# CarluerJB/3D_SIFT_CUDA

Measured on AMD Instinct MI355X. Metric: keypoints/s (.key records per second; Gauss-pyramid GB/s vs HBM roofline in `pyramid`/`roofline`), higher is better.
Workload: dtype f32

## Files before the change

### 3d_sift_cuda_amd/csrc/kernels_keypoint.hip

```cpp
#include <cstddef>
#include <type_traits>

#include "sift3d_internal.h"

#define PD SIFT3D_PATCH_DIM
#define PV SIFT3D_PATCH_VOX


__device__ __forceinline__ void interp_coord(float fX, float fMin, float fMax, int &ix, float &w)
{
    if (fX < fMin + 0.5f) {
        ix = (int)fMin;
        w = 1.0f;
    } else if (fX >= fMax - 0.5f) {
        ix = (int)(fMax - 2);
        w = 0.0f;
    } else {
        float mh = fX - 0.5f;
        ix = (int)floorf(mh);
        w = 1.0f - (mh - ((float)ix));
    }
}

__device__ __forceinline__ float trilinear(const float *__restrict__ img, int X, int XP, int Y, int Z, int Zl, int z_off,
                                           float x, float y, float z)
{
    float wx, wy, wz;
    int ix, iy, iz;
    interp_coord(x, 0, (float)X, ix, wx);
    interp_coord(y, 0, (float)Y, iy, wy);
    interp_coord(z, 0, (float)Z, iz, wz);
    iz -= z_off;
    iz = iz < 0 ? 0 : (iz > Zl - 2 ? Zl - 2 : iz);
    const long long XY = (long long)XP * Y;
    const float *p = img + (long long)iz * XY + (long long)iy * XP + ix;
    typedef float f2u __attribute__((ext_vector_type(2), aligned(4)));
    const f2u q00 = *reinterpret_cast<const f2u *>(p), q10 = *reinterpret_cast<const f2u *>(p + XP);
    const f2u q01 = *reinterpret_cast<const f2u *>(p + XY), q11 = *reinterpret_cast<const f2u *>(p + XY + XP);
    const float f000 = q00.x, f100 = q00.y, f010 = q10.x, f110 = q10.y;
    const float f001 = q01.x, f101 = q01.y, f011 = q11.x, f111 = q11.y;
    float fn00 = wx * f000 + (1.0f - wx) * f100;
    float fn01 = wx * f001 + (1.0f - wx) * f101;
    float fn10 = wx * f010 + (1.0f - wx) * f110;
    float fn11 = wx * f011 + (1.0f - wx) * f111;
    float fnn0 = wy * fn00 + (1.0f - wy) * fn10;
    float fnn1 = wy * fn01 + (1.0f - wy) * fn11;
    return wz * fnn0 + (1.0f - wz) * fnn1;
}

__device__ __forceinline__ double finddet(double a1, double a2, double a3, double b1, double b2, double b3, double c1,
                                          double c2, double c3)
{
    return ((a1 * b2 * c3) - (a1 * b3 * c2) - (a2 * b1 * c3) + (a3 * b1 * c2) + (a2 * b3 * c1) - (a3 * b2 * c1));
}
__device__ __forceinline__ double interp_quadratic(double x0, double x1, double x2, double fx0, double fx1, double fx2)
{
    if (!(fx1 < fx0 && fx1 < fx2) && !(fx1 > fx0 && fx1 > fx2)) return x1;
    double a1 = x0 * x0, b1 = x0, c1 = 1;
    double a2 = x1 * x1, b2 = x1, c2 = 1;
    double a3 = x2 * x2, b3 = x2, c3 = 1;
    double d1 = fx0, d2 = fx1, d3 = fx2;
    double det = finddet(a1, a2, a3, b1, b2, b3, c1, c2, c3);
    double detx = finddet(d1, d2, d3, b1, b2, b3, c1, c2, c3);
    double dety = finddet(a1, a2, a3, d1, d2, d3, c1, c2, c3);
    if (d1 == 0 && d2 == 0 && d3 == 0) return x1;
    if (det != 0) {
        if (detx != 0) return dety / (-2.0 * detx);
    }
    return x1;
}

__device__ __forceinline__ void invert3(const float *in, float *out)
{
    float a11 = in[0], a21 = in[3], a31 = in[6];
    float a12 = in[1], a22 = in[4], a32 = in[7];
    float a13 = in[2], a23 = in[5], a33 = in[8];
    float det = a11 * (a33 * a22 - a32 * a23) - a21 * (a33 * a12 - a32 * a13) + a31 * (a23 * a12 - a22 * a13);
    double div = 1 / (double)det;
    out[0] = (float)((a33 * a22 - a32 * a23) * div);
    out[3] = (float)(-(a33 * a21 - a31 * a23) * div);
    out[6] = (float)((a32 * a21 - a31 * a22) * div);
    out[1] = (float)(-(a33 * a12 - a32 * a13) * div);
    out[4] = (float)((a33 * a11 - a31 * a13) * div);
    out[7] = (float)(-(a32 * a11 - a31 * a12) * div);
    out[2] = (float)((a23 * a12 - a22 * a13) * div);
    out[5] = (float)(-(a23 * a11 - a21 * a13) * div);
    out[8] = (float)((a22 * a11 - a21 * a12) * div);
}

__device__ __forceinline__ void v3_norm(float *p)
{
    float ss = p[0] * p[0] + p[1] * p[1] + p[2] * p[2];
    if (ss > 0) {
        float div = (float)(1.0 / (double)sqrtf(ss));
        p[0] *= div;
        p[1] *= div;
        p[2] *= div;
    } else {
        p[0] = 1;
        p[1] = 0;
        p[2] = 0;
    }
}
__device__ __forceinline__ float v3_mag(const float *p)
{
    float ss = p[0] * p[0] + p[1] * p[1] + p[2] * p[2];
    if (ss > 0) return sqrtf(ss);
    return 0;
}
__device__ __forceinline__ float v3_dot(const float *a, const float *b) { return a[0] * b[0] + a[1] * b[1] + a[2] * b[2]; }

__device__ __forceinline__ double svd_with_sign(double magnitude, double sign_source) { return sign_source >= 0.0 ? fabs(magnitude) : -fabs(magnitude); }
__device__ __forceinline__ double svd_hypot(double p, double q) { return sqrt(p * p + q * q); }

__device__ __forceinline__ void svd3(float a[3][3], float w[3], float v[3][3])
{
    double off[3];
    double g = 0.0, scale = 0.0, norm = 0.0, s, f, h;
    int below = 0;

    for (int i = 0; i < 3; i++) {
        below = i + 1;
        off[i] = scale * g;
        g = s = scale = 0.0;
        for (int k = i; k < 3; k++) scale += fabsf(a[k][i]);
        if (scale) {
            for (int k = i; k < 3; k++) {
                a[k][i] = (float)(a[k][i] / scale);
                s += a[k][i] * a[k][i];
            }
            f = a[i][i];
            g = -svd_with_sign(sqrt(s), f);
            h = f * g - s;
            a[i][i] = (float)(f - g);
            for (int j = below; j < 3; j++) {
                s = 0.0;
                for (int k = i; k < 3; k++) s += a[k][i] * a[k][j];
                f = s / h;
                for (int k = i; k < 3; k++) a[k][j] = (float)(a[k][j] + f * a[k][i]);
            }
            for (int k = i; k < 3; k++) a[k][i] = (float)(a[k][i] * scale);
        }
        w[i] = (float)(scale * g);
        g = s = scale = 0.0;
        if (i != 2) {
            for (int k = below; k < 3; k++) scale += fabsf(a[i][k]);
            if (scale) {
                for (int k = below; k < 3; k++) {
                    a[i][k] = (float)(a[i][k] / scale);
                    s += a[i][k] * a[i][k];
                }
                f = a[i][below];
                g = -svd_with_sign(sqrt(s), f);
                h = f * g - s;
                a[i][below] = (float)(f - g);
                for (int k = below; k < 3; k++) off[k] = a[i][k] / h;
                for (int j = below; j < 3; j++) {
                    s = 0.0;
                    for (int k = below; k < 3; k++) s += a[j][k] * a[i][k];
                    for (int k = below; k < 3; k++) a[j][k] = (float)(a[j][k] + s * off[k]);
                }
                for (int k = below; k < 3; k++) a[i][k] = (float)(a[i][k] * scale);
            }
        }
        const double row_norm = fabsf(w[i]) + fabs(off[i]);
        norm = norm > row_norm ? norm : row_norm;
    }

    for (int i = 2; i >= 0; i--) {
        if (i < 2) {
            if (g) {
                for (int j = below; j < 3; j++) v[j][i] = (float)((a[i][j] / a[i][below]) / g);
                for (int j = below; j < 3; j++) {
                    s = 0.0;
                    for (int k = below; k < 3; k++) s += a[i][k] * v[k][j];
                    for (int k = below; k < 3; k++) v[k][j] = (float)(v[k][j] + s * v[k][i]);
                }
            }
            for (int j = below; j < 3; j++) v[i][j] = v[j][i] = 0.0;
        }
        v[i][i] = 1.0;
        g = off[i];
        below = i;
    }

    for (int i = 2; i >= 0; i--) {
        below = i + 1;
        g = w[i];
        for (int j = below; j < 3; j++) a[i][j] = 0.0;
        if (g) {
            g = 1.0 / g;
            for (int j = below; j < 3; j++) {
                s = 0.0;
                for (int k = below; k < 3; k++) s += a[k][i] * a[k][j];
                f = (s / a[i][i]) * g;
                for (int k = i; k < 3; k++) a[k][j] = (float)(a[k][j] + f * a[k][i]);
            }
            for (int j = i; j < 3; j++) a[j][i] = (float)(a[j][i] * g);
        } else {
            for (int j = i; j < 3; j++) a[j][i] = 0.0;
        }
        a[i][i] = a[i][i] + 1;
    }

    for (int k = 2; k >= 0; k--) {
        for (int sweep = 1; sweep <= 30; sweep++) {
            bool cancel = true;
            int lo = k, above = 0;
            for (; lo >= 0; lo--) {
                above = lo - 1;
                if ((double)(fabs(off[lo]) + norm) == norm) {
                    cancel = false;
                    break;
                }
                if ((double)(fabsf(w[above]) + norm) == norm) break;
            }
            double c, x, y, z;
            if (cancel) {
                c = 0.0;
                s = 1.0;
                for (int i = lo; i <= k; i++) {
                    f = s * off[i];
                    off[i] = c * off[i];
                    if ((double)(fabs(f) + norm) == norm) break;
                    g = w[i];
                    h = svd_hypot(f, g);
                    w[i] = (float)h;
                    h = 1.0 / h;
                    c = g * h;
                    s = -f * h;
                    for (int j = 0; j < 3; j++) {
                        y = a[j][above];
                        z = a[j][i];
                        a[j][above] = (float)(y * c + z * s);
                        a[j][i] = (float)(z * c - y * s);
                    }
                }
            }
            z = w[k];
            if (lo == k) {
                if (z < 0.0) {
                    w[k] = (float)(-z);
                    for (int j = 0; j < 3; j++) v[j][k] = -v[j][k];
                }
                break;
            }
            x = w[lo];
            above = k - 1;
            y = w[above];
            g = off[above];
            h = off[k];
            f = ((y - z) * (y + z) + (g - h) * (g + h)) / (2.0 * h * y);
            g = svd_hypot(f, 1.0);
            f = ((x - z) * (x + z) + h * ((y / (f + svd_with_sign(g, f))) - h)) / x;
            c = s = 1.0;
            for (int j = lo; j <= above; j++) {
                const int i = j + 1;
                g = off[i];
                y = w[i];
                h = s * g;
                g = c * g;
                z = svd_hypot(f, h);
                off[j] = z;
                c = f / z;
                s = h / z;
                f = x * c + g * s;
                g = g * c - x * s;
                h = y * s;
                y *= c;
                for (int r = 0; r < 3; r++) {
                    x = v[r][j];
                    z = v[r][i];
                    v[r][j] = (float)(x * c + z * s);
                    v[r][i] = (float)(z * c - x * s);
                }
                z = svd_hypot(f, h);
                w[j] = (float)z;
                if (z) {
                    z = 1.0 / z;
                    c = f * z;
                    s = h * z;
                }
                f = c * g + s * y;
                x = c * y - s * g;
                for (int r = 0; r < 3; r++) {
                    y = a[r][j];
                    z = a[r][i];
                    a[r][j] = (float)(y * c + z * s);
                    a[r][i] = (float)(z * c - y * s);
                }
            }
            off[lo] = 0.0;
            off[k] = f;
            w[k] = (float)x;
        }
    }
}
__device__ __forceinline__ void sort_eig(float w[3], float v[3][3])
{
    float t;
    for (int i = 0; i < 3; i++)
        for (int j = i + 1; j < 3; j++)
            if (w[i] < w[j]) {
                t = w[j]; w[j] = w[i]; w[i] = t;
                for (int k = 0; k < 3; k++) {
                    t = v[k][j]; v[k][j] = v[k][i]; v[k][i] = t;
                }
            }
}
typedef float v4f __attribute__((ext_vector_type(4)));
#define KP_NT 256
#define DESC_NT 128
#define NRAD 515
#define NRAD_PAD 516
#define NINT 729

template <int NT>
__device__ __forceinline__ void wave_sample_patch(float *patch, const float *__restrict__ img, int X, int XP, int Y, int Z, int Zl,
                                                  int z_off, float fx, float fy, float fz, float scale, const float *ori9)
{
    float inv[9];
    invert3(ori9, inv);
    const float rad = 2.0f * scale;
    const int sr = PD / 2;
    const float sc = rad / (float)(sr);
    int ax_fast = 0, ax_mid = 1, ax_slow = 2;
    {
        const float f0 = fabsf(inv[0]), f1 = fabsf(inv[1]), f2 = fabsf(inv[2]);
        ax_fast = f0 >= f1 && f0 >= f2 ? 0 : (f1 >= f2 ? 1 : 2);
        const int r0 = ax_fast == 0 ? 1 : 0, r1 = ax_fast == 2 ? 1 : 2;
        const bool first = fabsf(inv[3 + r0]) >= fabsf(inv[3 + r1]);
        ax_mid = first ? r0 : r1;
        ax_slow = first ? r1 : r0;
    }
    const int st_fast = ax_fast == 0 ? 1 : (ax_fast == 1 ? PD : PD * PD), st_mid = ax_mid == 0 ? 1 : (ax_mid == 1 ? PD : PD * PD),
              st_slow = ax_slow == 0 ? 1 : (ax_slow == 1 ? PD : PD * PD);
    for (int s0 = threadIdx.x; s0 < PV; s0 += 3 * NT) {
        float pix[3];
        int sidx[3];
#pragma unroll
        for (int u = 0; u < 3; u++) {
            const int t = s0 + NT * u;
            pix[u] = 0;
            sidx[u] = 0;
            if (t < PV) {
                const int s = (t % PD) * st_fast + ((t / PD) % PD) * st_mid + (t / (PD * PD)) * st_slow;
                sidx[u] = s;
                const int xx = s % PD - sr, yy = (s / PD) % PD - sr, zz = s / (PD * PD) - sr;
                float in3[3] = {(float)xx, (float)yy, (float)zz};
                float o[3];
#pragma unroll
                for (int i = 0; i < 3; i++) {
                    float a = 0;
#pragma unroll
                    for (int j = 0; j < 3; j++) a += inv[i * 3 + j] * in3[j];
                    o[i] = a;
                }
                o[0] *= sc; o[1] *= sc; o[2] *= sc;
                o[0] += fx; o[1] += fy; o[2] += fz;
                if (o[0] < 0 || o[0] >= X) pix[u] = 0;
                else pix[u] = trilinear(img, X, XP, Y, Z, Zl, z_off, o[0], o[1], o[2]);
            }
        }
#pragma unroll
        for (int u = 0; u < 3; u++)
            if (s0 + NT * u < PV) patch[sidx[u]] = pix[u];
    }
    __syncthreads();
}

template <bool SQUARE>
__device__ __forceinline__ float serial_sum_patch(const float *d)
{
    float acc = 0;
    const v4f *d4 = reinterpret_cast<const v4f *>(d);
    v4f a[8], b[8];
    auto add_block = [&](const v4f(&blk)[8]) {
#pragma unroll
        for (int q = 0; q < 8; q++) {
            const v4f v = blk[q];
            if (SQUARE) {
                acc += v.x * v.x; acc += v.y * v.y; acc += v.z * v.z; acc += v.w * v.w;
            } else {
                acc += v.x; acc += v.y; acc += v.z; acc += v.w;
            }
        }
    };
#pragma unroll
    for (int q = 0; q < 8; q++) a[q] = d4[q];
    for (int blk = 0; blk + 1 < 41; blk += 2) {
#pragma unroll
        for (int q = 0; q < 8; q++) b[q] = d4[(blk + 1) * 8 + q];
        add_block(a);
#pragma unroll
        for (int q = 0; q < 8; q++) a[q] = d4[(blk + 2) * 8 + q];
        add_block(b);
    }
    add_block(a);
    for (int i = 41 * 32; i < PV; i++) acc += SQUARE ? d[i] * d[i] : d[i];
    return acc;
}

template <int NT>
__device__ __forceinline__ void wave_normalize_patch(float *d, float *scratch2)
{
    if (threadIdx.x == 0) scratch2[0] = serial_sum_patch<false>(d) / (PD * PD * PD);
    __syncthreads();
    const float mean = scratch2[0];
    for (int i = threadIdx.x; i < PV; i += NT) d[i] -= mean;
    __syncthreads();
    if (threadIdx.x == 0) scratch2[1] = 1.0f / sqrtf(serial_sum_patch<true>(d));
    __syncthreads();
    const float div = scratch2[1];
    for (int i = threadIdx.x; i < PV; i += NT) d[i] *= div;
    __syncthreads();
}

__device__ __forceinline__ bool in_radius(int s)
{
    const int x = s % PD - PD / 2, y = (s / PD) % PD - PD / 2, z = s / (PD * PD) - PD / 2;
    const float fx = (float)x, fy = (float)y, fz = (float)z;
    return fz * fz + fy * fy + fx * fx < (float)((PD / 2) * (PD / 2));
}

__device__ __forceinline__ int wave_build_radius_list(unsigned short *rlist, int *n_lds)
{
    if (threadIdx.x < 64) {
        int n = 0;
        for (int base = 0; base < PV; base += 64) {
            const int s = base + threadIdx.x;
            const bool in = s < PV && in_radius(s);
            const unsigned long long m = __ballot(in);
            if (in) rlist[n + __popcll(m & ((1ull << threadIdx.x) - 1ull))] = (unsigned short)s;
            n += __popcll(m);
        }
        if (threadIdx.x == 0) *n_lds = n;
    }
    __syncthreads();
    return *n_lds;
}

template <int NT>
__device__ __forceinline__ void blur_pass(const float *src, float *dst, int axis, const float *taps, int ntaps)
{
    const int h = ntaps / 2;
    const int st = axis == 0 ? 1 : (axis == 1 ? PD : PD * PD);
    float tp[5], w[5];
#pragma unroll
    for (int j = 0; j < 5; j++) tp[j] = j < ntaps ? taps[j] : 0.0f;
    for (int ln = threadIdx.x; ln < PD * PD; ln += NT) {
        const int base = axis == 0 ? ln * PD : (axis == 1 ? (ln / PD) * PD * PD + ln % PD : ln);
#pragma unroll
        for (int j = 0; j < 5; j++) {
            const int pos = j - h;
            w[j] = (j < ntaps && pos >= 0 && pos < PD) ? src[base + pos * st] : 0.0f;
        }
#pragma unroll
        for (int c = 0; c < PD; c++) {
            float acc = 0;
#pragma unroll
            for (int j = 0; j < 5; j++) {
                const int cc = c + j - h;
                if (j < ntaps && cc >= 0 && cc < PD) acc = acc + tp[j] * w[j];
            }
            dst[base + c * st] = acc;
            const int nx = c + 1 + h;
            const float in = nx < PD ? src[base + nx * st] : 0.0f;
#pragma unroll
            for (int j = 0; j < 4; j++) w[j] = w[j + 1];
            if (ntaps >= 1) w[ntaps - 1 < 4 ? ntaps - 1 : 4] = in;
        }
    }
    __syncthreads();
}
template <int NT>
__device__ __forceinline__ void wave_blur_patch(float *in, float *tmp_a, float *tmp_b, const float *taps, int ntaps)
{
    blur_pass<NT>(in, tmp_a, 0, taps, ntaps);
    blur_pass<NT>(tmp_a, tmp_b, 1, taps, ntaps);
    blur_pass<NT>(tmp_b, tmp_a, 2, taps, ntaps);
}

template <int NT>
__device__ __forceinline__ int wave_peaks_sorted(const float *g, unsigned char *flags, int *n_lds, short *raw_idx, float *raw_val,
                                                 short *pk_idx, float *pk_val)
{
    static_assert(NT >= 81 + PD * PD, "one thread per interior row plus one per row for the border flags");
    const int t = threadIdx.x;
    if (t < 81) {
        const int y = t % 9 + 1, z = t / 9 + 1;
        const int rb = (z * PD + y) * PD;
        float a[9], b[9];
#pragma unroll
        for (int k = 0; k < 9; k++) {
            const int off = rb + ((k / 3 - 1) * PD + (k % 3 - 1)) * PD;
            a[k] = g[off];
            b[k] = g[off + 1];
        }
        flags[rb] = 0;
#pragma unroll
        for (int x = 1; x < PD - 1; x++) {
            float n[9];
#pragma unroll
            for (int k = 0; k < 9; k++) n[k] = g[rb + ((k / 3 - 1) * PD + (k % 3 - 1)) * PD + x + 1];
            const float c = b[4];
            bool pk = true;
#pragma unroll
            for (int k = 0; k < 9; k++) {
                pk = pk && (a[k] < c) && (n[k] < c);
                if (k != 4) pk = pk && (b[k] < c);
            }
            flags[rb + x] = pk ? 1 : 0;
#pragma unroll
            for (int k = 0; k < 9; k++) {
                a[k] = b[k];
                b[k] = n[k];
            }
        }
        flags[rb + PD - 1] = 0;
    } else if (t < 81 + PD * PD) {
        const int q = t - 81, y = q % PD, z = q / PD;
        if (y == 0 || y == PD - 1 || z == 0 || z == PD - 1) {
#pragma unroll
            for (int x = 0; x < PD; x++) flags[(z * PD + y) * PD + x] = 0;
        }
    }
    __syncthreads();
    if (threadIdx.x < 64) {
        int n = 0;
        for (int base = 0; base < PV; base += 64) {
            const int s = base + threadIdx.x;
            const bool pk = s < PV && flags[s] != 0;
            const unsigned long long m = __ballot(pk);
            if (pk) {
                const int pos = n + __popcll(m & ((1ull << threadIdx.x) - 1ull));
                raw_idx[pos] = (short)s;
                raw_val[pos] = g[s];
            }
            n += __popcll(m);
        }
        if (threadIdx.x == 0) *n_lds = n;
    }
    __syncthreads();
    const int n = *n_lds;
    for (int i = threadIdx.x; i < n; i += NT) {
        const float vi = raw_val[i];
        int rank = 0;
        for (int j = 0; j < n; j++) {
            const float vj = raw_val[j];
            rank += (vj > vi || (vj == vi && j < i)) ? 1 : 0;
        }
        pk_idx[rank] = raw_idx[i];
        pk_val[rank] = vi;
    }
    __syncthreads();
    return n;
}

__device__ __forceinline__ void interp_point_patch(const float *g, int s, float *o)
{
    const int ix = s % PD, iy = (s / PD) % PD, iz = s / (PD * PD);
    const float c = g[s];
    o[0] = (float)interp_quadratic(ix - 1, ix, ix + 1, g[s - 1], c, g[s + 1]);
    o[1] = (float)interp_quadratic(iy - 1, iy, iy + 1, g[s - PD], c, g[s + PD]);
    o[2] = (float)interp_quadratic(iz - 1, iz, iz + 1, g[s - PD * PD], c, g[s + PD * PD]);
}

__device__ __forceinline__ void splat_params(float x, float y, float z, short &base, float &wx, float &wy, float &wz)
{
    int ix, iy, iz;
    interp_coord(x, 0, (float)PD, ix, wx);
    interp_coord(y, 0, (float)PD, iy, wy);
    interp_coord(z, 0, (float)PD, iz, wz);
    base = (short)(ix | (iy << 4) | (iz << 8));
}

__device__ __forceinline__ void wave_splat_sequence(float *grid, int n, const short *sp_base, const v4f *sp4)
{
    const int lane = threadIdx.x;
    const int slot = lane >> 3;
    const int a = lane & 1, b = (lane >> 1) & 1, c = (lane >> 2) & 1;
    float *g = grid;
    if (lane < 64) {
        int packed = 0;
        float wx = 0, wy = 0, wz = 0, v = 0;
        if (slot < n) {
            packed = sp_base[slot];
            const v4f q = sp4[slot];
            wx = q.x; wy = q.y; wz = q.z; v = q.w;
        }
        for (int g0 = 0; g0 < n; g0 += 8) {
            const int i = g0 + slot;
            const bool ok = i < n;
            const int ix = packed & 15, iy = (packed >> 4) & 15, iz = packed >> 8;
            const int cell = ((iz + c) * PD + (iy + b)) * PD + (ix + a);
            const float ux = a ? (1.0f - wx) : wx;
            const float uy = b ? (1.0f - wy) : wy;
            const float uz = c ? (1.0f - wz) : wz;
            const float contrib = v * ux * uy * uz;
            const int in = i + 8;
            if (in < n) {
                packed = sp_base[in];
                const v4f q = sp4[in];
                wx = q.x; wy = q.y; wz = q.z; v = q.w;
            }
#pragma unroll
            for (int j = 0; j < 8; j++) {
                if (slot == j && ok) __hip_atomic_fetch_add(&g[cell], contrib, __ATOMIC_RELAXED, __HIP_MEMORY_SCOPE_WORKGROUP);
                __builtin_amdgcn_wave_barrier();
            }
        }
    }
    __syncthreads();
}

__device__ __forceinline__ long long xcd_contiguous_item(long long n, int seg)
{
    const long long b = blockIdx.x;
    if (seg <= 0) {
        const long long per = (n + 7) / 8;
        return (b % 8) * per + b / 8;
    }
    const long long s0 = b / seg * seg, local = b - s0;
    return s0 + (local % 8) * (seg / 8) + local / 8;
}

struct kpA_smem {
    float A[PV + 1];
    union {
        float sp_tail[2 * NRAD_PAD];
        struct {
            unsigned char flags[PV + 13];
            short raw_idx[128], pk2_idx[128];
            float raw_val[128], pk2_val[128];
        } pk;
    } C;
    float B[PV + 1];
    float gx[NRAD_PAD], gy[NRAD_PAD], gz[NRAD_PAD];
    union {
        unsigned short rlist[NRAD_PAD];
        short sp_base[NRAD_PAD];
    } r;
    short pk_idx[128];
    float pk_val[128];
    float ori_data[PD * 3 + 3];
    float sc[16];
    float taps[8];
    int cnt[4];
};
static_assert(sizeof(kpA_smem) * 7 <= 160 * 1024, "seven workgroups per CU");
static_assert(offsetof(kpA_smem, C) == sizeof(float) * (PV + 1) && sizeof(float) * (PV + 1) + sizeof(float) * 2 * NRAD_PAD >= 16 * NRAD_PAD,
              "the splat parameters span A and C");

__global__ __launch_bounds__(KP_NT, 7) void keypoint_kernel(sift3d_kp_params p, const unsigned long long *__restrict__ keys,
                                                      const sift3d_cval *__restrict__ vals, long long ncand,
                                                      sift3d_dkp *__restrict__ kps, int *__restrict__ nrec_out,
                                                      sift3d_taps taps3)
{
    __shared__ __attribute__((aligned(16))) kpA_smem sm;
    const long long k = blockIdx.x;
    if (k >= ncand) return;
    const int lane = threadIdx.x;
    if (lane < 3) sm.taps[lane] = taps3.f[lane];
    const unsigned long long key = keys[k];
    const sift3d_cval cvl = vals[k];
    const int lvl = (int)(key >> SIFT3D_KEY_LVL_SHIFT);
    const int is_max = (int)((key >> SIFT3D_KEY_MAX_SHIFT) & 1ull);
    const long long cidx = (long long)(key & SIFT3D_KEY_IDX_MASK);
    const sift3d_level lv = p.levels[lvl];
    sift3d_dkp *kp = kps + k;
    const int X = lv.X, Y = lv.Y, Z = lv.Z, XP = lv.XP;
    const long long XY = (long long)XP * Y;
    const int ix = (int)(cidx % XP), iy = (int)((cidx / XP) % Y), iz = (int)(cidx / XY) + lv.z_off;

    const float *C = lv.dogc;
    const float cv = C[cidx];
    float fx = (float)interp_quadratic(ix - 1, ix, ix + 1, C[cidx - 1], cv, C[cidx + 1]);
    float fy = (float)interp_quadratic(iy - 1, iy, iy + 1, C[cidx - XP], cv, C[cidx + XP]);
    float fz = (float)interp_quadratic(iz - 1, iz, iz + 1, C[cidx - XY], cv, C[cidx + XY]);
    float scale = (float)(2 * interp_quadratic(lv.sigma_h, lv.sigma_c, lv.sigma_l, cvl.h, cv, cvl.l));
    fx += 0.5f; fy += 0.5f; fz += 0.5f;

    const float rad = 2.0f * scale;
    const int rmax = (int)(rad + 2);
    if (fx - rmax < 0 || fy - rmax < 0 || fz - rmax < 0 || fx + rmax >= X || fy + rmax >= Y || fz + rmax >= Z) {
        if (lane == 0) nrec_out[k] = 0;
        return;
    }
    float *patch = sm.A;
    const float ident[9] = {1, 0, 0, 0, 1, 0, 0, 0, 1};
    wave_sample_patch<KP_NT>(patch, lv.img, X, lv.XP, Y, Z, lv.Zl, lv.z_off, fx, fy, fz, scale, ident);
#ifdef SIFT3D_DEV
    if (p.debug_stop == 1) { if (lane == 0) nrec_out[k] = 0; return; }
#endif
    wave_normalize_patch<KP_NT>(patch, sm.sc);
#ifdef SIFT3D_DEV
    if (p.debug_stop == 2) { if (lane == 0) nrec_out[k] = 0; return; }
#endif
    const int nrad = wave_build_radius_list(sm.r.rlist, &sm.cnt[0]);

    for (int i = lane; i < NRAD_PAD; i += KP_NT) {
        float a = 0, b = 0, c = 0;
        if (i < nrad) {
            const int s = sm.r.rlist[i];
            a = patch[s + 1] - patch[s - 1];
            b = patch[s + PD] - patch[s - PD];
            c = patch[s + PD * PD] - patch[s - PD * PD];
        }
        sm.gx[i] = a; sm.gy[i] = b; sm.gz[i] = c;
    }
    __syncthreads();
    if (lane < 9) {
        const float *ei = lane / 3 == 0 ? sm.gx : (lane / 3 == 1 ? sm.gy : sm.gz);
        const float *ej = lane % 3 == 0 ? sm.gx : (lane % 3 == 1 ? sm.gy : sm.gz);
        float acc = 0;
        int i = 0;
        for (; i + 16 <= nrad; i += 16) {
            v4f a[4], b[4];
#pragma unroll
            for (int q = 0; q < 4; q++) {
                a[q] = *reinterpret_cast<const v4f *>(ei + i + 4 * q);
                b[q] = *reinterpret_cast<const v4f *>(ej + i + 4 * q);
            }
#pragma unroll
            for (int q = 0; q < 4; q++) {
                acc += a[q].x * b[q].x; acc += a[q].y * b[q].y; acc += a[q].z * b[q].z; acc += a[q].w * b[q].w;
            }
        }
        for (; i < nrad; i++) acc += ei[i] * ej[i];
        sm.sc[lane] = acc;
    }
    __syncthreads();
#ifdef SIFT3D_DEV
    if (p.debug_stop == 3) { if (lane == 0) nrec_out[k] = 0; return; }
#endif
    auto svd_and_eigen_test = [&]() {
        float mat[3][3], w[3], v[3][3];
        for (int i = 0; i < 3; i++)
            for (int j = 0; j < 3; j++) {
                mat[i][j] = sm.sc[i * 3 + j];
                v[i][j] = 0;
            }
        w[0] = w[1] = w[2] = 0;
        svd3(mat, w, v);
        sort_eig(w, v);
        float es = w[0] + w[1] + w[2];
        float ep = w[0] * w[1] * w[2];
        float esp = es * es * es;
        int keep = (esp < p.eig_thres * ep || p.eig_thres < 0) ? 1 : 0;
        sm.sc[15] = keep ? 1.0f : 0.0f;
        if (keep) {
            kp->x = fx; kp->y = fy; kp->z = fz; kp->scale = scale;
            kp->eigs[0] = w[0]; kp->eigs[1] = w[1]; kp->eigs[2] = w[2];
            for (int i = 0; i < 3; i++)
                for (int j = 0; j < 3; j++) kp->ori0[i * 3 + j] = v[i][j];
            kp->info = is_max ? SIFT3D_INFO_MIN0MAX1 : 0u;
            kp->lvl = lvl;
        } else {
            nrec_out[k] = 0;
        }
    };
#ifdef SIFT3D_DEV
    const bool svd_first = p.debug_stop == 40;
    if (svd_first) {
        if (lane == KP_NT - 64) svd_and_eigen_test();
        __syncthreads();
        if (sm.sc[15] == 0.0f) return;
    }
#else
    constexpr bool svd_first = false;
#endif
    for (int s = lane; s < PV; s += KP_NT) p.patch0[(long long)k * PV + s] = patch[s];
    __syncthreads();

    float *t0 = sm.B;
    float *ta = sm.A;
    v4f *sp4 = reinterpret_cast<v4f *>(sm.A);
    const float radius = (float)(PD / 2);
    for (int s = lane; s < PV; s += KP_NT) t0[s] = 0;
    for (int i = lane; i < nrad; i += KP_NT) {
        float e[3] = {sm.gx[i], sm.gy[i], sm.gz[i]};
        float m2 = e[0] * e[0] + e[1] * e[1] + e[2] * e[2];
        float mg = 0, wx = 0, wy = 0, wz = 0;
        short base = 0;
        if (m2 != 0) {
            mg = sqrtf(m2);
            float u[3];
            for (int q = 0; q < 3; q++) u[q] = e[q] * radius / mg;
            for (int q = 0; q < 3; q++) u[q] += radius;
            splat_params((float)(u[0] + 0.5), (float)(u[1] + 0.5), (float)(u[2] + 0.5), base, wx, wy, wz);
        }
        sm.r.sp_base[i] = base;
        v4f q; q.x = wx; q.y = wy; q.z = wz; q.w = mg;
        sp4[i] = q;
    }
    __syncthreads();
    if (!svd_first && lane == KP_NT - 64) svd_and_eigen_test();
    wave_splat_sequence(t0, nrad, sm.r.sp_base, sp4);
    if (sm.sc[15] == 0.0f) return;
#ifdef SIFT3D_DEV
    if (p.debug_stop == 4 || p.debug_stop == 5) { if (lane == 0) nrec_out[k] = 0; return; }
#endif
#ifdef SIFT3D_DEV
    if (p.debug_stop == 6) { if (lane == 0) nrec_out[k] = 0; return; }
#endif
    wave_blur_patch<KP_NT>(t0, ta, t0, sm.taps, 3);
#ifdef SIFT3D_DEV
    if (p.debug_stop == 7) { if (lane == 0) nrec_out[k] = 0; return; }
#endif
    const int npk = wave_peaks_sorted<KP_NT>(ta, sm.C.pk.flags, &sm.cnt[1], sm.C.pk.raw_idx, sm.C.pk.raw_val, sm.pk_idx, sm.pk_val);
#ifdef SIFT3D_DEV
    if (p.debug_stop == 8) { if (lane == 0) nrec_out[k] = 0; return; }
#endif

    if (lane < npk && lane < PD && lane < 30) {
        float o[3];
        interp_point_patch(ta, sm.pk_idx[lane], o);
        o[0] -= radius; o[1] -= radius; o[2] -= radius;
        v3_norm(o);
        sm.ori_data[lane * 3 + 0] = o[0];
        sm.ori_data[lane * 3 + 1] = o[1];
        sm.ori_data[lane * 3 + 2] = o[2];
    }
    __syncthreads();

    int nret = 0;
    const float pk0 = npk > 0 ? sm.pk_val[0] : 0.0f;
    for (int i = 0; i < npk && i < PD && nret < 30; i++) {
        if ((double)sm.pk_val[i] < 0.8 * (double)pk0) break;
        const float p1[3] = {sm.ori_data[i * 3], sm.ori_data[i * 3 + 1], sm.ori_data[i * 3 + 2]};
        __syncthreads();
        for (int s = lane; s < PV; s += KP_NT) t0[s] = 0;
        for (int q = lane; q < nrad; q += KP_NT) {
            float e[3] = {sm.gx[q], sm.gy[q], sm.gz[q]};
            float mg = v3_mag(e);
            float wx = 0, wy = 0, wz = 0;
            short base = 0;
            if (mg != 0) {
                float u[3] = {e[0], e[1], e[2]};
                v3_norm(u);
                float par = v3_dot(p1, u);
                float pp[3];
                pp[0] = u[0] - par * p1[0];
                pp[1] = u[1] - par * p1[1];
                pp[2] = u[2] - par * p1[2];
                v3_norm(pp);
                for (int r = 0; r < 3; r++) {
                    pp[r] *= radius;
                    pp[r] += radius;
                }
                splat_params((float)(pp[0] + 0.5), (float)(pp[1] + 0.5), (float)(pp[2] + 0.5), base, wx, wy, wz);
            }
            sm.r.sp_base[q] = base;
            v4f pq; pq.x = wx; pq.y = wy; pq.z = wz; pq.w = mg;
            sp4[q] = pq;
        }
        __syncthreads();
#ifdef SIFT3D_DEV
        if (p.debug_stop == 31) { if (lane == 0) nrec_out[k] = 0; return; }
#endif
        wave_splat_sequence(t0, nrad, sm.r.sp_base, sp4);
#ifdef SIFT3D_DEV
        if (p.debug_stop == 32) { if (lane == 0) nrec_out[k] = 0; return; }
#endif
        wave_blur_patch<KP_NT>(t0, ta, t0, sm.taps, 3);
#ifdef SIFT3D_DEV
        if (p.debug_stop == 33) { if (lane == 0) nrec_out[k] = 0; return; }
#endif
        const int npk2 = wave_peaks_sorted<KP_NT>(ta, sm.C.pk.flags, &sm.cnt[2], sm.C.pk.raw_idx, sm.C.pk.raw_val, sm.C.pk.pk2_idx, sm.C.pk.pk2_val);
#ifdef SIFT3D_DEV
        if (p.debug_stop == 34) { if (lane == 0) nrec_out[k] = 0; return; }
#endif
        const float pk20 = npk2 > 0 ? sm.C.pk.pk2_val[0] : 0.0f;
        for (int j = 0; j < npk2 && nret < PD && nret < 30; j++) {
            if (sm.C.pk.pk2_val[j] < 0.5f * pk20) break;
            if (lane == 0) {
                float p2[3], p3[3];
                interp_point_patch(ta, sm.C.pk.pk2_idx[j], p2);
                p2[0] -= radius; p2[1] -= radius; p2[2] -= radius;
                v3_norm(p2);
                float par = v3_dot(p1, p2);
                p2[0] = p2[0] - par * p1[0];
                p2[1] = p2[1] - par * p1[1];
                p2[2] = p2[2] - par * p1[2];
                v3_norm(p2);
                p3[0] = p1[1] * p2[2] - p1[2] * p2[1];
                p3[1] = -p1[0] * p2[2] + p1[2] * p2[0];
                p3[2] = p1[0] * p2[1] - p1[1] * p2[0];
                float *m = kp->frames + 9 * nret;
                for (int iv = 0; iv < 3; iv++) {
                    m[0 * 3 + iv] = p1[iv];
                    m[1 * 3 + iv] = p2[iv];
                    m[2 * 3 + iv] = p3[iv];
                }
            }
            nret++;
        }
    }
    if (lane == 0) {
        kp->nframes = nret;
        nrec_out[k] = 1 + nret;
    }
}

__device__ __forceinline__ float lane_value(float x, int i)
{
    return __builtin_bit_cast(float, __builtin_amdgcn_readlane(__builtin_bit_cast(int, x), i));
}

__constant__ unsigned char c_brief_x[192] = {
    5,4,4,4,4,2,6,5,5,4,4,4,3,8,5,5,6,3,5,5,5,5,6,5,4,6,6,6,3,4,4,4,5,3,4,5,4,5,5,4,2,7,7,5,3,5,4,5,3,5,7,3,5,5,2,3,5,5,6,6,4,6,5,4,
    4,6,5,3,5,6,4,3,6,4,4,5,3,3,3,6,6,5,2,4,4,6,3,6,3,2,3,5,4,5,3,4,3,6,5,4,3,6,4,5,2,4,3,7,2,3,6,5,2,6,3,3,5,6,3,6,3,5,3,6,5,7,4,2,
    5,5,5,2,5,7,4,2,5,3,4,3,3,7,4,4,7,6,4,4,2,8,7,6,5,4,7,3,6,6,5,2,4,5,3,2,5,5,1,6,3,6,3,6,2,5,4,4,7,2,6,3,2,2,4,3,3,2,3,4,2,5,6,7};
__constant__ unsigned char c_brief_y[192] = {
    6,5,3,4,5,3,7,4,6,4,3,2,4,7,5,3,5,1,5,4,7,6,8,4,4,5,6,5,2,5,4,6,4,0,4,3,3,4,4,2,1,7,8,6,4,4,1,6,1,3,7,2,3,3,1,3,6,1,6,6,4,7,6,4,
    3,5,4,2,3,6,4,5,6,3,3,5,1,3,1,6,7,4,1,4,3,5,2,4,2,1,2,5,4,5,2,3,3,3,3,4,2,6,3,4,3,3,3,6,1,2,5,4,2,4,1,4,6,7,3,6,2,4,3,6,5,6,4,0,
    6,6,5,1,4,7,2,1,5,3,4,2,2,7,3,3,6,4,2,4,1,9,7,7,5,2,7,1,7,5,5,1,5,4,1,3,3,4,0,5,1,6,3,5,3,2,3,3,7,2,5,1,1,0,4,1,3,1,0,3,1,6,5,9};

struct kpB_sift {
    float mag[NINT + 3];
    unsigned short order[NINT + 3];
    unsigned char bin[NINT + 3];
    int start[9];
};
struct kpB_brief {
    float t1[PV + 1];
};
template <bool SIFT>
struct kpB_smem {
    float patch[PV + 1];
    struct {
        typename std::conditional<SIFT, kpB_sift, kpB_brief>::type v;
    } u;
    float sc[16];
    float taps[8];
    float wtab[2][PD + 1];
};

template <bool SIFT>
__global__ __launch_bounds__(DESC_NT) void descriptor_kernel(sift3d_kp_params p, const sift3d_dkp *__restrict__ kps,
                                                        const int *__restrict__ rec_kp, const int *__restrict__ rec_frame,
                                                        long long nrec, sift3d_feature *__restrict__ recs,
                                                        int *__restrict__ rec_group, sift3d_taps taps5)
{
    __shared__ __attribute__((aligned(16))) kpB_smem<SIFT> sm;
    const long long r = xcd_contiguous_item(nrec, p.desc_seg);
    if (r >= nrec) return;
    const int lane = threadIdx.x;
    if (lane < 5) sm.taps[lane] = taps5.f[lane];
    const sift3d_dkp *kp = kps + rec_kp[r];
    const int fr = rec_frame[r];
    float ori[9];
    if (fr < 0) {
        ori[0] = 1; ori[1] = 0; ori[2] = 0; ori[3] = 0; ori[4] = 1; ori[5] = 0; ori[6] = 0; ori[7] = 0; ori[8] = 1;
    } else {
        for (int i = 0; i < 9; i++) ori[i] = kp->frames[fr * 9 + i];
    }
    const sift3d_level lv = p.levels[kp->lvl];
#ifdef SIFT3D_DEV
    if (p.debug_stop >= 21 && p.debug_stop <= 26) {
        wave_sample_patch<DESC_NT>(sm.patch, lv.img, lv.X, lv.XP, lv.Y, lv.Z, lv.Zl, lv.z_off, 20.0f, 20.0f, 20.0f, 3.0f, ori);
        if (p.debug_stop == 21) return;
    } else
#endif
    if (fr < 0) {
        const float *src = p.patch0 + (long long)rec_kp[r] * PV;
        for (int s = lane; s < PV; s += DESC_NT) sm.patch[s] = src[s];
        __syncthreads();
    } else {
        int *tok = nullptr;
        if (p.sampler_cap > 0) {
            unsigned hw, xcc;
            asm volatile("s_getreg_b32 %0, hwreg(HW_REG_HW_ID)" : "=s"(hw));
            asm volatile("s_getreg_b32 %0, hwreg(HW_REG_XCC_ID)" : "=s"(xcc));
            tok = p.sampler_tokens + ((((xcc & 7u) * 8u + ((hw >> 13) & 7u)) * 2u + ((hw >> 12) & 1u)) * 16u + ((hw >> 8) & 15u));
            if (lane == 0) {
                for (int tries = 0;; tries++) {
                    if (atomicAdd(tok, 1) < p.sampler_cap || tries > 50000) break;
                    atomicSub(tok, 1);
                    __builtin_amdgcn_s_sleep(64);
                }
            }
            __syncthreads();
        }
        wave_sample_patch<DESC_NT>(sm.patch, lv.img, lv.X, lv.XP, lv.Y, lv.Z, lv.Zl, lv.z_off, kp->x, kp->y, kp->z, kp->scale, ori);
        if (tok && lane == 0) atomicSub(tok, 1);
    }
#ifdef SIFT3D_DEV
    if (p.debug_stop == 11) return;
#endif
    wave_normalize_patch<DESC_NT>(sm.patch, sm.sc);
#ifdef SIFT3D_DEV
    if (p.debug_stop == 12 || p.debug_stop == 23) return;
#endif

    const bool w0 = lane < 64;
    float myval = 0.0f;
    if constexpr (SIFT) {
        for (int q = lane; q < NINT; q += DESC_NT) {
            const int x = q % 9 + 1, y = (q / 9) % 9 + 1, z = q / 81 + 1;
            const int s = (z * PD + y) * PD + x;
            float e[3] = {sm.patch[s + 1] - sm.patch[s - 1], sm.patch[s + PD] - sm.patch[s - PD],
                          sm.patch[s + PD * PD] - sm.patch[s - PD * PD]};
            float mg = v3_mag(e);
            int best = 8;
            if (mg > 0) {
                v3_norm(e);
                const float oa[8][3] = {{1, 1, 1},  {1, 1, -1},  {1, -1, 1},  {1, -1, -1},
                                        {-1, 1, 1}, {-1, 1, -1}, {-1, -1, 1}, {-1, -1, -1}};
                best = 0;
                float bd = v3_dot(oa[0], e);
#pragma unroll
                for (int t = 1; t < 8; t++) {
                    float d = v3_dot(oa[t], e);
                    if (d > bd) {
                        bd = d;
                        best = t;
                    }
                }
            }
            sm.u.v.mag[q] = mg;
            sm.u.v.bin[q] = (unsigned char)best;
        }
        if (lane < PD) {
            const float binsz = PD / (float)2;
            const int c = lane;
            float v = (int)(c / binsz) + 0.5f;
            if ((int)((c + 0) / binsz) != (int)((c + 1) / binsz)) {
                float p0 = ((c + 0) / binsz);
                float p1 = ((c + 1) / binsz);
                v = (p0 + p1) / 2.0f;
            }
            float w;
            int i0;
            interp_coord(v, 0, 2.0f, i0, w);
            sm.wtab[0][c] = w;
            sm.wtab[1][c] = 1.0f - w;
        }
        __syncthreads();
#ifdef SIFT3D_DEV
        if (p.debug_stop == 13 || p.debug_stop == 24) return;
#endif
        if (w0) {
            int cnt[8];
#pragma unroll
            for (int o = 0; o < 8; o++) cnt[o] = 0;
            for (int base = 0; base < NINT; base += 64) {
                const int q = base + lane;
                const int b = q < NINT ? sm.u.v.bin[q] : 8;
#pragma unroll
                for (int o = 0; o < 8; o++) cnt[o] += __popcll(__ballot(b == o));
            }
            int run[8];
            int acc0 = 0;
#pragma unroll
            for (int o = 0; o < 8; o++) {
                run[o] = acc0;
                if (lane == 0) sm.u.v.start[o] = acc0;
                acc0 += cnt[o];
            }
            if (lane == 0) sm.u.v.start[8] = acc0;
            for (int base = 0; base < NINT; base += 64) {
                const int q = base + lane;
                const int b = q < NINT ? sm.u.v.bin[q] : 8;
#pragma unroll
                for (int o = 0; o < 8; o++) {
                    const unsigned long long m = __ballot(b == o);
                    if (b == o) {
                        const int x = q % 9 + 1, y = (q / 9) % 9 + 1, z = q / 81 + 1;
                        sm.u.v.order[run[o] + __popcll(m & ((1ull << lane) - 1ull))] = (unsigned short)(x | (y << 4) | (z << 8));
                    }
                    run[o] += __popcll(m);
                }
            }
        }
        __syncthreads();
#ifdef SIFT3D_DEV
        if (p.debug_stop == 14 || p.debug_stop == 25) return;
#endif
        if (w0) {
            const int o = lane & 7, bx = (lane >> 3) & 1, by = (lane >> 4) & 1, bz = (lane >> 5) & 1;
            const float *wxs = sm.wtab[bx], *wys = sm.wtab[by], *wzs = sm.wtab[bz];
            const int k0 = sm.u.v.start[o], k1 = sm.u.v.start[o + 1];
            float acc = 0;
            for (int kk = k0; kk < k1; kk++) {
                const unsigned v = sm.u.v.order[kk];
                const int x = v & 15, y = (v >> 4) & 15, z = v >> 8;
                const float mg = sm.u.v.mag[((z - 1) * 9 + (y - 1)) * 9 + (x - 1)];
                acc += mg * wxs[x] * wys[y] * wzs[z];
            }
#ifdef SIFT3D_DEV
            if (p.debug_stop == 26) return;
#endif
            float mn = 100000;
#pragma unroll
            for (int i = 0; i < 64; i++) {
                float vi = lane_value(acc, i);
                if (vi < mn) mn = vi;
            }
            float v = acc - mn;
            float ss = 0;
#pragma unroll
            for (int i = 0; i < 64; i++) {
                float vi = lane_value(v, i);
                ss += vi * vi;
            }
            float div = 1.0f / sqrtf(ss);
            myval = v * div;
        }
    } else {
        wave_blur_patch<DESC_NT>(sm.patch, sm.u.v.t1, sm.patch, sm.taps, 5);
        if (w0) {
            const float *bl = sm.u.v.t1;
            const int x1 = c_brief_x[3 * lane], y1 = c_brief_x[3 * lane + 1], z1 = c_brief_x[3 * lane + 2];
            const int x2 = c_brief_y[3 * lane], y2 = c_brief_y[3 * lane + 1], z2 = c_brief_y[3 * lane + 2];
            float d = bl[x1 + y1 * PD + z1 * PD * PD] - bl[x2 + y2 * PD + z2 * PD * PD];
            if (p.desc_mode == SIFT3D_DESC_BRIEF) {
                myval = (d < 0) ? 1.0f : 0.0f;
            } else if (p.desc_mode == SIFT3D_DESC_RRIEF) {
                myval = d;
            } else {
                float fdx = x1 - x2, fdy = y1 - y2, fdz = z1 - z2;
                int dist = (int)sqrtf(fdx * fdx + fdy * fdy + fdz * fdz);
                myval = d / dist;
            }
        }
    }
    if (!w0) return;
    int rank = 0;
#pragma unroll
    for (int j = 0; j < 64; j++) {
        float vj = lane_value(myval, j);
        rank += (vj < myval || (vj == myval && j < lane)) ? 1 : 0;
    }
    const int grp = kp->lvl * 2 + ((kp->info & SIFT3D_INFO_MIN0MAX1) ? 1 : 0);
    sift3d_feature *out = recs + r + (p.rec_shift ? (long long)p.rec_shift[grp] : 0ll);
    out->desc[lane] = (float)rank;
    static_assert(offsetof(sift3d_feature, desc) == 17 * 4 && offsetof(sift3d_feature, ori) == 16 && offsetof(sift3d_feature, eigs) == 52 &&
                      offsetof(sift3d_feature, info) == 64, "record layout: x y z scale ori[9] eigs[3] info desc[64]");
    if (lane < 17) {
        const float fac = lv.octave_factor, add = 0;
        unsigned word;
        if (lane < 4) {
            float v = lane == 0 ? kp->x : (lane == 1 ? kp->y : (lane == 2 ? kp->z : kp->scale));
            if (lane == 3) v *= fac;
            else v = v * fac + add;
            v *= p.size_factor;
            word = __builtin_bit_cast(unsigned, v);
        } else if (lane < 13) {
            word = __builtin_bit_cast(unsigned, fr < 0 ? kp->ori0[lane - 4] : kp->frames[fr * 9 + lane - 4]);
        } else if (lane < 16) {
            word = __builtin_bit_cast(unsigned, kp->eigs[lane - 13]);
        } else {
            word = kp->info | (fr < 0 ? 0u : SIFT3D_INFO_REORIENT);
        }
        reinterpret_cast<unsigned *>(out)[lane] = word;
        if (lane == 0) rec_group[r] = grp;
    }
}

__global__ void group_count_kernel(const unsigned long long *__restrict__ keys, const int *__restrict__ nrec, long long ncand, int *__restrict__ counts)
{
    const long long k = (long long)blockIdx.x * blockDim.x + threadIdx.x;
    if (k >= ncand) return;
    const int n = nrec[k];
    if (n <= 0) return;
    int g = (int)(keys[k] >> SIFT3D_KEY_LVL_SHIFT) * 2 + (int)((keys[k] >> SIFT3D_KEY_MAX_SHIFT) & 1ull);
    if (g < 0 || g >= SIFT3D_GROUPS - 1) g = SIFT3D_GROUPS - 1;
    atomicAdd(counts + g, n);
}

hipError_t sift3d_launch_group_counts(hipStream_t s, const unsigned long long *keys, const int *nrec, int64_t ncand, int *counts)
{
    if (ncand <= 0) return hipSuccess;
    hipLaunchKernelGGL(group_count_kernel, dim3((unsigned)((ncand + 255) / 256)), dim3(256), 0, s, keys, nrec, (long long)ncand, counts);
    return hipGetLastError();
}

__global__ void recmap_kernel(const int *__restrict__ nrec, const int *__restrict__ offs, long long ncand, int cand_off,
                              int *rec_base, int *__restrict__ rec_kp, int *__restrict__ rec_frame, unsigned long long *kp_count)
{
    const long long k = (long long)blockIdx.x * blockDim.x + threadIdx.x;
    if (k >= ncand) return;
    const int n = nrec[k], o = rec_base[0] + offs[k];
    if (k == ncand - 1) rec_base[1] = o + n;
    if (n > 0) atomicAdd(kp_count, 1ull);
    for (int f = 0; f < n; f++) {
        rec_kp[o + f] = cand_off + (int)k;
        rec_frame[o + f] = f - 1;
    }
}

hipError_t sift3d_launch_keypointsA(hipStream_t s, const sift3d_kp_params &p, const unsigned long long *keys,
                                    const sift3d_cval *vals, int64_t ncand, sift3d_dkp *kps, int *nrec, const float *taps3)
{
    if (ncand <= 0) return hipSuccess;
    sift3d_taps t;
    for (int i = 0; i < 17; i++) t.f[i] = i < 3 ? taps3[i] : 0.0f;
    hipLaunchKernelGGL(keypoint_kernel, dim3((unsigned)ncand), dim3(KP_NT), 0, s, p, keys, vals, (long long)ncand, kps, nrec, t);
    return hipGetLastError();
}

hipError_t sift3d_launch_recmap(hipStream_t s, const int *nrec, const int *offs, int64_t ncand, int cand_off, int *rec_base,
                                int *rec_kp, int *rec_frame, unsigned long long *kp_count)
{
    if (ncand <= 0) return hipSuccess;
    hipLaunchKernelGGL(recmap_kernel, dim3((unsigned)((ncand + 255) / 256)), dim3(256), 0, s, nrec, offs, (long long)ncand,
                       cand_off, rec_base, rec_kp, rec_frame, kp_count);
    return hipGetLastError();
}

hipError_t sift3d_launch_descriptors(hipStream_t s, const sift3d_kp_params &p, const sift3d_dkp *kps, const int *rec_kp,
                                     const int *rec_frame, int64_t nrec, sift3d_feature *recs, int *rec_group,
                                     const float *taps5)
{
    if (nrec <= 0) return hipSuccess;
    sift3d_taps t;
    for (int i = 0; i < 17; i++) t.f[i] = i < 5 ? taps5[i] : 0.0f;
    const int seg = p.desc_seg;
    const dim3 grid((unsigned)(seg > 0 ? (nrec + seg - 1) / seg * seg : ((nrec + 7) / 8) * 8));
    if (p.desc_mode == SIFT3D_DESC_SIFT)
        hipLaunchKernelGGL(descriptor_kernel<true>, grid, dim3(DESC_NT), 0, s, p, kps, rec_kp, rec_frame, (long long)nrec, recs,
                           rec_group, t);
    else
        hipLaunchKernelGGL(descriptor_kernel<false>, grid, dim3(DESC_NT), 0, s, p, kps, rec_kp, rec_frame, (long long)nrec, recs,
                           rec_group, t);
    return hipGetLastError();
}
```

Baseline: 18.63 million.

## Bucket descriptor terms per sub-box using nonzero weight coords and precompute products

The per-orientation ordering of all interior voxels is replaced by eight sub-box passes. Each pass enumerates only the coordinates whose interpolation weight is nonzero for that sub-box and writes the premultiplied mag*weight products into a compacted terms array reused from the patch buffer. The final accumulation then becomes a plain per-lane segment sum with fewer dependent LDS loads, and the lanes no longer iterate over voxels whose weight is zero. The cost is a more complex wave-serial bucketing step with division-based index decoding, and the patch buffer is overwritten.

```diff
diff --git a/3d_sift_cuda_amd/csrc/kernels_keypoint.hip b/3d_sift_cuda_amd/csrc/kernels_keypoint.hip
--- a/3d_sift_cuda_amd/csrc/kernels_keypoint.hip
+++ b/3d_sift_cuda_amd/csrc/kernels_keypoint.hip
@@ -919,9 +919,10 @@
 
 struct kpB_sift {
     float mag[NINT + 3];
-    unsigned short order[NINT + 3];
     unsigned char bin[NINT + 3];
-    int start[9];
+    unsigned char nzc[2][12];
+    int nnz[2];
+    int lst[65];
 };
 struct kpB_brief {
     float t1[PV + 1];
@@ -1034,61 +1035,92 @@
             float w;
             int i0;
             interp_coord(v, 0, 2.0f, i0, w);
+            const float w1 = 1.0f - w;
             sm.wtab[0][c] = w;
-            sm.wtab[1][c] = 1.0f - w;
+            sm.wtab[1][c] = w1;
+            const bool in = c >= 1 && c <= PD - 2;
+            const unsigned long long lt = (1ull << lane) - 1ull;
+            const unsigned long long m0 = __ballot(in && w != 0.0f), m1 = __ballot(in && w1 != 0.0f);
+            if (in && w != 0.0f) sm.u.v.nzc[0][__popcll(m0 & lt)] = (unsigned char)c;
+            if (in && w1 != 0.0f) sm.u.v.nzc[1][__popcll(m1 & lt)] = (unsigned char)c;
+            if (lane == 0) {
+                sm.u.v.nnz[0] = __popcll(m0);
+                sm.u.v.nnz[1] = __popcll(m1);
+            }
         }
         __syncthreads();
 #ifdef SIFT3D_DEV
         if (p.debug_stop == 13 || p.debug_stop == 24) return;
 #endif
+        float *terms = sm.patch;
         if (w0) {
-            int cnt[8];
-#pragma unroll
-            for (int o = 0; o < 8; o++) cnt[o] = 0;
-            for (int base = 0; base < NINT; base += 64) {
-                const int q = base + lane;
-                const int b = q < NINT ? sm.u.v.bin[q] : 8;
-#pragma unroll
-                for (int o = 0; o < 8; o++) cnt[o] += __popcll(__ballot(b == o));
-            }
-            int run[8];
-            int acc0 = 0;
-#pragma unroll
-            for (int o = 0; o < 8; o++) {
-                run[o] = acc0;
-                if (lane == 0) sm.u.v.start[o] = acc0;
-                acc0 += cnt[o];
-            }
-            if (lane == 0) sm.u.v.start[8] = acc0;
-            for (int base = 0; base < NINT; base += 64) {
-                const int q = base + lane;
-                const int b = q < NINT ? sm.u.v.bin[q] : 8;
+            const unsigned long long lt = (1ull << lane) - 1ull;
+            int tot = 0;
+            for (int s = 0; s < 8; s++) {
+                const int bx = s & 1, by = (s >> 1) & 1, bz = s >> 2;
+                const int nx = sm.u.v.nnz[bx], nxy = nx * sm.u.v.nnz[by], nbox = nxy * sm.u.v.nnz[bz];
+                const float rnx = 1.0f / (float)nx, rnxy = 1.0f / (float)nxy;
+                auto voxel = [&](int i, int &x, int &y, int &z) {
+                    const int iz = (int)(((float)i + 0.5f) * rnxy), r = i - iz * nxy;
+                    const int iy = (int)(((float)r + 0.5f) * rnx), ix = r - iy * nx;
+                    x = sm.u.v.nzc[bx][ix];
+                    y = sm.u.v.nzc[by][iy];
+                    z = sm.u.v.nzc[bz][iz];
+                };
+                int cnt[8];
+#pragma unroll
+                for (int o = 0; o < 8; o++) cnt[o] = 0;
+                for (int i0 = 0; i0 < nbox; i0 += 64) {
+                    int b = 8;
+                    if (i0 + lane < nbox) {
+                        int x, y, z;
+                        voxel(i0 + lane, x, y, z);
+                        b = sm.u.v.bin[((z - 1) * 9 + (y - 1)) * 9 + (x - 1)];
+                    }
+#pragma unroll
+                    for (int o = 0; o < 8; o++) cnt[o] += __popcll(__ballot(b == o));
+                }
+                int run[8];
 #pragma unroll
                 for (int o = 0; o < 8; o++) {
-                    const unsigned long long m = __ballot(b == o);
-                    if (b == o) {
-                        const int x = q % 9 + 1, y = (q / 9) % 9 + 1, z = q / 81 + 1;
-                        sm.u.v.order[run[o] + __popcll(m & ((1ull << lane) - 1ull))] = (unsigned short)(x | (y << 4) | (z << 8));
+                    run[o] = tot;
+                    if (lane == 0) sm.u.v.lst[s * 8 + o] = tot;
+                    tot += cnt[o];
+                }
+                for (int i0 = 0; i0 < nbox; i0 += 64) {
+                    int b = 8, x = 0, y = 0, z = 0;
+                    if (i0 + lane < nbox) {
+                        voxel(i0 + lane, x, y, z);
+                        b = sm.u.v.bin[((z - 1) * 9 + (y - 1)) * 9 + (x - 1)];
                     }
-                    run[o] += __popcll(m);
-                }
-            }
+                    int pos = 0;
+#pragma unroll
+                    for (int o = 0; o < 8; o++) {
+                        const unsigned long long m = __ballot(b == o);
+                        if (b == o) pos = run[o] + __popcll(m & lt);
+                        run[o] += __popcll(m);
+                    }
+                    if (b < 8 && pos < PV) {
+                        const float mg = sm.u.v.mag[((z - 1) * 9 + (y - 1)) * 9 + (x - 1)];
+                        terms[pos] = mg * sm.wtab[bx][x] * sm.wtab[by][y] * sm.wtab[bz][z];
+                    }
+                }
+            }
+            if (lane == 0) sm.u.v.lst[64] = tot;
         }
         __syncthreads();
 #ifdef SIFT3D_DEV
         if (p.debug_stop == 14 || p.debug_stop == 25) return;
 #endif
         if (w0) {
-            const int o = lane & 7, bx = (lane >> 3) & 1, by = (lane >> 4) & 1, bz = (lane >> 5) & 1;
-            const float *wxs = sm.wtab[bx], *wys = sm.wtab[by], *wzs = sm.wtab[bz];
-            const int k0 = sm.u.v.start[o], k1 = sm.u.v.start[o + 1];
+            const int k0 = sm.u.v.lst[lane], k1 = sm.u.v.lst[lane + 1];
             float acc = 0;
-            for (int kk = k0; kk < k1; kk++) {
-                const unsigned v = sm.u.v.order[kk];
-                const int x = v & 15, y = (v >> 4) & 15, z = v >> 8;
-                const float mg = sm.u.v.mag[((z - 1) * 9 + (y - 1)) * 9 + (x - 1)];
-                acc += mg * wxs[x] * wys[y] * wzs[z];
-            }
+            int kk = k0;
+            for (; kk + 4 <= k1; kk += 4) {
+                const float t0 = terms[kk], t1 = terms[kk + 1], t2 = terms[kk + 2], t3 = terms[kk + 3];
+                acc += t0; acc += t1; acc += t2; acc += t3;
+            }
+            for (; kk < k1; kk++) acc += terms[kk];
 #ifdef SIFT3D_DEV
             if (p.debug_stop == 26) return;
 #endif
```

Result: faster. 18.91 million, median of 6 (+1.5%).
